# quarkquartet/nuSIprop

Measured on AMD Instinct MI355X. Metric: full propagations/sec at N_E=300, 1 & 8 GPU; achieved HBM GB/s on cascade kernel, higher is better.
Workload: dtype f64

## Files before the change

nusiprop_amd/csrc/nusi_kernels.hip:

```cpp
#include <hip/hip_runtime.h>

#include <algorithm>
#include <cstdlib>
#include <vector>

#include "nusi_internal.hpp"

namespace nusi {


__device__ __attribute__((noinline)) void warn_entry(int* warn, int* wmin, int T, int p, int w, int n, int m)
{
    atomicOr(&warn[p], w);
    if (wmin)
#pragma unroll
        for (int b = 0; b < 4; ++b)
            if ((w >> b) & 1) atomicMin(&wmin[((size_t)p * 4 + b) * T + n], m);
}

constexpr int kGaWaves = 4;
constexpr int kGaTerms = kAlphatSlots;
struct LdsSink {
    double* v;
    double* r;
// ... 152 lines not shown
    if (n >= T) return;
    const Point& P = pts[p];
    if (!P.non_resonant) return;
    double v[2];
    int f;
    const int nv = ga_pre_slot(P, k, g.lo[n], g.hi[n], slot, v, &f);
    double* o = pre + ((size_t)(p * 3 + k) * kGaPreFields + f) * T + n;
    o[0] = v[0];
    if (nv == 2) o[T] = v[1];
}

size_t gamma_alphat_pre_doubles(int T, int npts) { return (size_t)3 * kGaPreFields * T * npts; }

hipError_t launch_gamma_alphat(const GridDev& g, const Point* pts, int npts, const SplineSet* spl, TablesDev t,
                               int* warn, hipStream_t s, bool ref)
{
    dim3 grid((g.T + 62) / 63, npts, 2);
    if (ref && t.Gpre) {
        hipLaunchKernelGGL(k_ga_dilogs, dim3((g.T + 63) / 64, npts, 3 * kGaPreSlots), dim3(64), 0, s, g, pts, t.Gpre);
        hipLaunchKernelGGL((k_gamma_alphat<true, 2, true>), grid, dim3(384), 0, s, g, pts, spl, t.G, t.At, warn, t.Wmin,
                           t.Gpre);
        return hipGetLastError();
    }
    if (npts <= 16) {
        if (ref) hipLaunchKernelGGL((k_gamma_alphat<true, 2>), grid, dim3(384), 0, s, g, pts, spl, t.G, t.At, warn, t.Wmin);
        else hipLaunchKernelGGL((k_gamma_alphat<false, 2>), grid, dim3(384), 0, s, g, pts, spl, t.G, t.At, warn, t.Wmin);
    } else {
        if (ref) hipLaunchKernelGGL((k_gamma_alphat<true, 1>), grid, dim3(192), 0, s, g, pts, spl, t.G, t.At, warn, t.Wmin);
        else hipLaunchKernelGGL((k_gamma_alphat<false, 1>), grid, dim3(192), 0, s, g, pts, spl, t.G, t.At, warn, t.Wmin);
    }
    return hipGetLastError();
}


__host__ __device__ constexpr int alpha_tile_lds_doubles(int cs, int ct, int G)
{
    return alpha_tile_corner_block(cs, ct, G) + alpha_tile_edge_doubles(cs, ct, G) + (G > 1 ? G * kTileThreads : 0);
}

constexpr int kTileWaves = 3;
#define NUSI_TILE_ATTR __attribute__((amdgpu_waves_per_eu(kTileWaves, kTileWaves)))
template <int G, bool kRef>
__global__ __launch_bounds__(kTileThreads) NUSI_TILE_ATTR void k_alpha_tile(GridDev g, const Point* __restrict__ pts, const SplineSet* __restrict__ splp,
                                                           const int* __restrict__ tiles, int cs_max, int ct_max,
                                                           const int* __restrict__ batches,
                                                           double* __restrict__ A, int* __restrict__ warn,
                                                           int* __restrict__ wmin)
{
    extern __shared__ __attribute__((aligned(16))) double sm[];
    const SplineSet& spl = *splp;
    __shared__ double tE[2 * kAlphaTile], sE[2 * kAlphaTile];
    __shared__ int tl[kAlphaTile], th[kAlphaTile], sl[kAlphaTile], sh[kAlphaTile];
    __shared__ int cnt[2];
    __shared__ double elo[2][kAlphaTile], ehi[2][kAlphaTile];
    const int tid = threadIdx.x, T = g.T;
    const int bw = batches ? batches[blockIdx.y] : (int)blockIdx.y | (1 << 24);
    const int p0 = bw & 0xffffff, nb = (G == 1) ? 1 : bw >> 24;
    const AlphaTile tile = alpha_tile_decode(tiles + kTileWords * blockIdx.x);
    const int n0 = tile.n0, m0 = tile.m0;
    const int Tm = (m0 + tile.mcnt < T) ? m0 + tile.mcnt : T;
    const int Tn = (n0 + tile.ncnt < T) ? n0 + tile.ncnt : T;
    const Point& P = pts[p0];
    if (tid < 2 * kAlphaTile) {
        const int side = tid / kAlphaTile, j = tid - side * kAlphaTile, b = (side ? m0 : n0) + j;
        if (b < (side ? Tm : Tn)) { elo[side][j] = g.lo[b]; ehi[side][j] = g.hi[b]; }
    }
    __syncthreads();
    if (tid == 0) cnt[0] = alpha_edge_list(elo[0], ehi[0], 0, Tn - n0, tE, tl, th);
    if (tid == 64) cnt[1] = alpha_edge_list(elo[1], ehi[1], 0, Tm - m0, sE, sl, sh);
    __syncthreads();
    const int ct = cnt[0], cs = cnt[1], cc = cs * ct;
    const int ln = tid % kAlphaTile, lm = tid / kAlphaTile;
    const int n = n0 + ln, m = m0 + lm;
    const bool valid = alpha_tile_slot_valid(tile, T, tid);
    if (cs > cs_max || ct > ct_max || nb > G) {
        if (valid)
            for (int q = 0; q < nb; ++q) A[(size_t)(p0 + q) * g.PT + (size_t)m * (m - 1) / 2 + n] = __builtin_nan("");
        return;
    }
    const bool nonres = P.non_resonant, maj = P.majorana;
    const bool needed = valid && (nonres || m == n + 1);
    double* cor = sm;
    double* edg = sm + alpha_tile_corner_block(cs, ct, G);
    double* tsum = edg + alpha_tile_edge_doubles(cs, ct, G);
    double tot1 = 0.0;
    {
        const int per = ct + cs + kAlphaTile, w = tid >> 6, l = tid & 63;
        int job = -1;
        if (3 * ct <= 64 && 3 * cs <= 128) {
            if (w == 0) { if (l < 3 * ct) job = (l / ct) * per + l % ct; }
            else if (w <= 2) { const int q = tid - 64; if (q < 3 * cs) job = (q / cs) * per + ct + q % cs; }
            else if (l < 3 * kAlphaTile) job = (l / kAlphaTile) * per + ct + cs + l % kAlphaTile;
        } else if (tid < 3 * per) {
            job = tid;
        }
        if (job >= 0) {
            alpha_tile_edge_job(P, job, tE, ct, sE, cs, g.lo, g.hi, m0, Tm, edg);
#pragma unroll 1
            for (int q = 0; q < nb; ++q)
                alpha_tile_edge_member_job(pts[p0 + q], q, G, job, tE, ct, sE, cs, g.lo, g.hi, m0, Tm, edg);
        }
        if (G > 1)
            for (int q = 0; q < nb; ++q) tsum[q * kTileThreads + tid] = 0.0;
    }
    for (int k = 0; k < 3; ++k) {
        __syncthreads();
        if (nonres && maj) {
            const double* edgk = edg + k * alpha_tile_edge_stride(cs, ct);
            for (int j = tid; j < cc; j += kTileThreads) {
                alpha_tile_corner_job<kRef>(j, edgk, ct, cs, cor);
#pragma unroll 1
                for (int q = 0; q < nb; ++q) alpha_tile_corner_member_job<kRef>(pts[p0 + q], q, j, edgk, ct, cs, cor);
            }
            for (int j = tid; j < kAlphaTile * (cs + ct); j += kTileThreads)
                alpha_tile_mixed_job(j, edgk, ct, cs, G, tl, th, sl, sh, n0, m0, Tn, Tm, cor);
        }
        __syncthreads();
        if (needed) {
            AlphaPre pre;
            const bool share = G > 1 && nb > 1 && nonres && maj;
            if (share) {
                const TileLeaves lv0 = alpha_tile_leaves(cor, edg, k, 0, G, cs, ct, lm, sl, sh, tl, th, ln);
                alpha_k_pre(P, k, g.lo[n], g.hi[n], g.lo[m], g.hi[m], lv0, pre);
            }
#pragma unroll 1
            for (int q = 0; q < nb; ++q) {
                double tot = (G > 1) ? tsum[q * kTileThreads + tid] : tot1;
                int w = 0;
                const TileLeaves lv = alpha_tile_leaves(cor, edg, k, q, G, cs, ct, lm, sl, sh, tl, th, ln);
                alpha_k(pts[p0 + q], spl, k, g.lo[n], g.hi[n], g.lo[m], g.hi[m], lv, tot, w, share ? &pre : nullptr);
                if (G > 1) tsum[q * kTileThreads + tid] = tot;
                else tot1 = tot;
                if (w) warn_entry(warn, wmin, T, p0 + q, w, n, m);
            }
        }
    }
    if (valid)
        for (int q = 0; q < nb; ++q)
            A[(size_t)(p0 + q) * g.PT + (size_t)m * (m - 1) / 2 + n] =
                needed ? ((G > 1) ? tsum[q * kTileThreads + tid] : tot1) : 0.0;
}

constexpr int kBatchQC = 5;
__host__ __device__ inline int alpha_batch_lds_doubles()
{
    const int c1 = kAlphaTile + 1;
    return (3 + kXFields + 2) * c1 * c1 + alpha_tile_edge_stride(c1, c1) +
           kBatchQC * alpha_batch_memb_doubles(c1, c1);
}
static_assert(kXFields * (kAlphaTile + 1) * (kAlphaTile + 1) >= 4 * (kAlphaTile + 1) * (kAlphaTile + 1) + kAlphaTile * 2 * (kAlphaTile + 1),
              "the bracket phase's blocks fit X");
static_assert(kBatchQC * (2 * (kAlphaTile + 1) + kAlphaTile) <= kTileThreads, "one member-edge round per chunk");
static_assert(3 + kBatchQC <= kXFields, "(kRef) the chunk's A fields fit X beside Dcr, Dci");

constexpr int kBatchWaves = 4, kBatchWavesRefo = 3;
constexpr int batch_waves(bool pp, bool ref) { return ref && !pp ? kBatchWavesRefo : kBatchWaves; }
#define NUSI_BCOLD __device__ __attribute__((noinline))
template <bool kRef>
NUSI_BCOLD void b_corner(int j, const double* edgk, int ct, int cs, double* per, double* tmp)
{
    alpha_batch_corner_job<kRef>(j, edgk, ct, cs, per, tmp);
}
NUSI_BCOLD double b_marg(double S, double t, double gr) { return alpha_member_ref_arg(S, t, gr); }
NUSI_BCOLD void b_xshared(int j, const double* edgk, int ct, int cs, double* X) { alpha_batch_xshared_job(j, edgk, ct, cs, X); }
NUSI_FN SplitLeaves batch_bracket_leaves(const double* P3, const double* tmp, const double* mix, const double* edgk,
                                         int cs, int ct, int lm, int ln, int s0, int s1, int t0, int t1)
{
    const int cc = cs * ct;
    SplitLeaves lv;
    lv.cf[0] = P3; lv.cf[1] = tmp; lv.cf[2] = tmp + kCC; lv.cf[3] = tmp + 2 * kCC; lv.cf[4] = tmp + 3 * kCC;
    lv.cf[5] = P3 + kCC; lv.cf[6] = P3 + 2 * kCC;
    lv.corm = P3;
    lv.cc = cc; lv.ct = ct; lv.cs = cs; lv.mb = lm; lv.nb = ln;
    lv.sidx[0] = s0; lv.sidx[1] = s1; lv.tidx[0] = t0; lv.tidx[1] = t1;
    lv.ted = edgk; lv.sed = edgk + kTEdgeFields * ct; lv.mbv = lv.sed + kSEdgeFields * cs;
    lv.tedm = P3; lv.sedm = P3; lv.mbm = P3; lv.marg = P3;
    lv.xl = mix; lv.yl = mix + kAlphaTile * cs;
    return lv;
}
NUSI_BCOLD AlphaPre b_pre(const Point& P, int k, double Em, double Ep, double Emp, double Epp, const double* P3,
                          const double* tmp, const double* mix, const double* edgk, int cs, int ct, int lm, int ln,
                          int s0, int s1, int t0, int t1)
{
    const SplitLeaves lv = batch_bracket_leaves(P3, tmp, mix, edgk, cs, ct, lm, ln, s0, s1, t0, t1);
    AlphaPre pre;
    alpha_k_pre(P, k, Em, Ep, Emp, Epp, lv, pre);
    return pre;
}

__global__ __launch_bounds__(256) void k_alpha_medge(GridDev g, const Point* __restrict__ pts, double* __restrict__ med)
{
    const int j = blockIdx.x * 256 + threadIdx.x, p = blockIdx.y, k = blockIdx.z, T = g.T;
    if (j >= 5 * T) return;
    alpha_medge_job(pts[p], k, j, T, g.lo, g.hi, med + ((size_t)p * 3 + k) * kMedFields * T);
}

constexpr int kMcJobs = 1024;
__global__ __launch_bounds__(256) void k_alpha_mcorner(const Point* __restrict__ pts, const int* __restrict__ batches,
                                                       MCornerDev mc, int pc0, int jobs)
{
    __shared__ double v[2 * kMcJobs];
    __shared__ double cst[2][kMcJobs];
    const int bw = batches[blockIdx.y], k = blockIdx.z, tid = threadIdx.x;
    const int p0 = bw & 0xffffff, nb = (int)((unsigned)bw >> 24);
    const Point& P = pts[p0];
    if (!(P.non_resonant && P.majorana)) return;
    const int cb = jobs / nb;
    const long long c0 = (long long)blockIdx.x * cb;
    if (c0 >= mc.NC) return;
    const int nj = cb * nb;
    for (int cl = tid; cl < cb && c0 + cl < mc.NC; cl += 256) alpha_mcorner_st(P, k, c0 + cl, mc.ue, cst[0][cl], cst[1][cl]);
    __syncthreads();
    for (int j = tid; j < nj; j += 256) {
        const int cl = j / nb, q = j - cl * nb;
        if (c0 + cl >= mc.NC) break;
        const double S = cst[0][cl], t = cst[1][cl], gr = pts[p0 + q].a_gr;
        const cd Dc = alpha_member_ref_dc_inl(S, t, gr);
        v[2 * (q * cb + cl)] = Dc.r;
        v[2 * (q * cb + cl) + 1] = Dc.i;
    }
    __syncthreads();
    double* const o = mc.buf + (size_t)(p0 - pc0) * 6 * mc.NC + (size_t)k * 2 * nb * mc.NC;
    for (int e = tid; e < 2 * nj; e += 256) {
        const int q = e / (2 * cb), r = e - q * 2 * cb;
        if (c0 + r / 2 < mc.NC) o[((size_t)q * mc.NC + c0) * 2 + r] = v[e];
    }
}

void mcorner_edges(int T, const double* lo, const double* hi, std::vector<int>& eu, std::vector<double>& ue)
{
    eu.assign(2 * (size_t)T, 0);
    ue.clear();
    for (int b = 0; b < T; ++b) {
        if (b == 0 || !(lo[b] == hi[b - 1])) ue.push_back(lo[b]);
        eu[2 * b] = (int)ue.size() - 1;
        ue.push_back(hi[b]);
        eu[2 * b + 1] = (int)ue.size() - 1;
    }
}


#ifdef NUSI_BATCH_TRACE
constexpr int kBtWg = 16, kBtN = 512;
__device__ unsigned long long g_bt[kBtWg * 4 * kBtN];
#define NUSI_BT()                                                                                                   \
    do {                                                                                                            \
        if (kRef && !kPP && !kSplit && kPair == 1 && blockIdx.x < 4 && blockIdx.y < 4 && (threadIdx.x & 63) == 0 && bt_i < kBtN) \
            g_bt[((blockIdx.y * 4 + blockIdx.x) * 4 + (threadIdx.x >> 6)) * kBtN + bt_i] = __builtin_amdgcn_s_memtime(); \
        ++bt_i;                                                                                                     \
    } while (0)
#else
#define NUSI_BT() do { } while (0)
#endif
template <bool kPP, bool kRef, bool kSplit, int kPair>
__device__ __forceinline__ void alpha_batch_body(const GridDev& g, const Point* __restrict__ pts, const SplineSet* __restrict__ splp,
                                                 const int* __restrict__ tiles, const int* __restrict__ batches,
                                                 double* __restrict__ A, const double* __restrict__ med,
                                                 int* __restrict__ warn, int* __restrict__ wmin, const MCornerDev& mc,
                                                 int pc0, double* __restrict__ kt)
{
    static_assert(kPair == 1 || (kPair == 2 && kRef && !kPP && !kSplit), "paired points: the reference order without phi-phi");
    constexpr int kQC = kPair == 2 ? 4 : kBatchQC;
    extern __shared__ __attribute__((aligned(16))) double sm[];
    const SplineSet& spl = *splp;
    __shared__ double tE[2 * kAlphaTile], sE[2 * kAlphaTile];
    __shared__ int tl[kAlphaTile], th[kAlphaTile], sl[kAlphaTile], sh[kAlphaTile];
    __shared__ int cnt[2];
    __shared__ double elo[2][kAlphaTile], ehi[2][kAlphaTile];
    __shared__ unsigned char elist[kPair == 2 ? kPairEntries : 1];
    const int tid = threadIdx.x, T = g.T;
    const int bx = blockIdx.x, by = blockIdx.y;
    const int bw = batches[by];
    const int p0 = bw & 0xffffff, nb = (int)((unsigned)bw >> 24);
    const AlphaTile tile = alpha_tile_decode(tiles + kTileWords * bx);
    const int n0 = tile.n0, m0 = tile.m0;
    const int Tm = (m0 + tile.mcnt < T) ? m0 + tile.mcnt : T;
    const int Tn = (n0 + tile.ncnt < T) ? n0 + tile.ncnt : T;
    const Point& P = pts[p0];
    if (kPair == 2) {
        const int r = alpha_tile_entry_rank(tile, T, tid);
        if (r >= 0 && r < kPairEntries) elist[r] = (unsigned char)tid;
    }
    if (tid < 2 * kAlphaTile) {
        const int side = tid / kAlphaTile, j = tid - side * kAlphaTile, b = (side ? m0 : n0) + j;
        if (b < (side ? Tm : Tn)) { elo[side][j] = g.lo[b]; ehi[side][j] = g.hi[b]; }
    }
    __syncthreads();
    if (tid == 0) cnt[0] = alpha_edge_list(elo[0], ehi[0], 0, Tn - n0, tE, tl, th);
    if (tid == 64) cnt[1] = alpha_edge_list(elo[1], ehi[1], 0, Tm - m0, sE, sl, sh);
    __syncthreads();
    const int ct = cnt[0], cs = cnt[1], cc = cs * ct;
    __shared__ int tsrc[2 * kAlphaTile], ssrc[2 * kAlphaTile];
    if (tid < 2 * kAlphaTile) {
        const int side = tid / kAlphaTile, j = tid - side * kAlphaTile, b0 = side ? m0 : n0;
        const int* il = side ? sl : tl;
        const int* ih = side ? sh : th;
        int* src = side ? ssrc : tsrc;
        if (b0 + j < (side ? Tm : Tn)) {
            src[ih[j]] = 2 * (b0 + j) + 1;
            if (j == 0 || il[j] != ih[j - 1]) src[il[j]] = 2 * (b0 + j);
        }
    }
    const int hq = kPair == 2 ? __builtin_amdgcn_readfirstlane(tid / kPairEntries) : 0;
    const int nent = kPair == 2 ? alpha_tile_entries(tile, T) : 0;
    int slot = tid;
    if (kPair == 2) {
        const int e = tid % kPairEntries;
        slot = (e < nent && nent <= kPairEntries) ? elist[e] : kTileThreads - 1;
    }
    const int ln = slot % kAlphaTile, lm = slot / kAlphaTile;
    const int n = n0 + ln, m = m0 + lm;
    const bool valid = alpha_tile_slot_valid(tile, T, slot);
    const size_t eidx = (size_t)m * (m - 1) / 2 + n;
    if (cs > kAlphaTile + 1 || ct > kAlphaTile + 1 || (kPair == 2 && nent > kPairEntries)) {
        if (alpha_tile_slot_valid(tile, T, tid)) {
            const int md = m0 + tid / kAlphaTile;
            for (int q = 0; q < nb; ++q)
                A[(size_t)(p0 + q) * g.PT + (size_t)md * (md - 1) / 2 + n0 + tid % kAlphaTile] = __builtin_nan("");
        }
        return;
    }
    const bool nonres = P.non_resonant, maj = P.majorana, cornered = nonres && maj;
    const bool needed = valid && (nonres || m == n + 1);
    constexpr int ccmax = kCC;
    double* P3 = sm;
    double* X = P3 + 3 * ccmax;
    double* mem = X + kXFields * ccmax;
    double* edgk = mem + 2 * ccmax;
    double* membq = edgk + alpha_tile_edge_stride(kAlphaTile + 1, kAlphaTile + 1);
    const int mbd = alpha_batch_memb_doubles(cs, ct);
    double* tmp = X;
    double* mix = X + 4 * kCC;
    const int mjobs = ct + cs + kAlphaTile;
    int wsh = 0;
    const int kb = kSplit ? (int)blockIdx.z : 0, ke = kSplit ? kb + 1 : 3;
#ifdef NUSI_BATCH_TRACE
    int bt_i = 0;
#endif
#pragma unroll 1
    for (int k = kb; k < ke; ++k) {
        NUSI_BT();
        __syncthreads();
        if (tid < mjobs) alpha_tile_edge_job_k(P, k, tid, tE, ct, sE, cs, g.lo, g.hi, m0, Tm, edgk);
        __syncthreads();
        NUSI_BT();
        AlphaPre pre{};
        PPTerm ppt{0.0, 1.0, 1.0};
        if (cornered) {
            for (int j = tid; j < cc; j += kTileThreads) b_corner<kRef>(j, edgk, ct, cs, P3, tmp);
            for (int j = tid; j < kAlphaTile * (cs + ct); j += kTileThreads)
                alpha_batch_mixed_job(j, edgk, ct, cs, tl, th, sl, sh, n0, m0, Tn, Tm, mix, mix + kAlphaTile * cs);
            __syncthreads();
            NUSI_BT();
            if (needed) {
                pre = b_pre(P, k, g.lo[n], g.hi[n], g.lo[m], g.hi[m], P3, tmp, mix, edgk, cs, ct, lm, ln, sl[lm], sh[lm],
                            tl[ln], th[ln]);
                if (kPP) {
                    const SplitLeaves lv = batch_bracket_leaves(P3, tmp, mix, edgk, cs, ct, lm, ln, sl[lm], sh[lm],
                                                                tl[ln], th[ln]);
                    ppt = alpha_k_pp(P, spl, k, g.lo[n], g.hi[n], g.lo[m], g.hi[m], lv, wsh);
                }
            }
            __syncthreads();
            NUSI_BT();
            if (!kRef)
                for (int j = tid; j < cc; j += kTileThreads) b_xshared(j, edgk, ct, cs, X);
        }
        const bool reload = !kSplit && k > 0 && needed;
        double tnext = reload && hq < nb ? A[(size_t)(p0 + hq) * g.PT + eidx] : 0.0;
        const int mq = tid / mjobs, mjob = tid - mq * mjobs;
        const double2* const mcb =
            kRef ? reinterpret_cast<const double2*>(mc.buf + (size_t)(p0 - pc0) * 6 * mc.NC + (size_t)k * 2 * nb * mc.NC)
                 : nullptr;
        int moff = -1;
        double2 mcv = make_double2(0.0, 0.0), mcv2 = mcv;
        if (kRef && cornered && tid < cc) {
            const int si = tid / ct, ti = tid - si * ct;
            const int us = mc.eu[ssrc[si]], ut = mc.eu[tsrc[ti]];
            if (ut <= us) {
                moff = us * (us + 1) / 2 + ut;
                mcv = mcb[moff];
                if (kPair == 2 && nb > 1) mcv2 = mcb[mc.NC + moff];
            }
        }
#pragma unroll 1
        for (int q0 = 0; q0 < nb; q0 += kQC) {
            const int nq = (nb - q0 < kQC) ? nb - q0 : kQC;
            __syncthreads();
            NUSI_BT();
            if (mq < nq) {
                MedVals mv{};
                alpha_batch_medge_load(nonres, mjob, tsrc, ct, ssrc, cs, m0, Tm, T,
                                       med + ((size_t)(p0 + q0 + mq) * 3 + k) * kMedFields * T, mv);
                alpha_batch_medge_store(nonres, mjob, ct, cs, m0, Tm, mv, membq + mq * mbd);
            }
            if (kRef && moff >= 0) {
                const int si = tid / ct, ti = tid - si * ct;
                const double S = edgk[kTEdgeFields * ct + kSEdgeVal * cs + si], t = edgk[kTEdgeVal * ct + ti];
#pragma unroll 1
                for (int qq = 0; qq < nq; ++qq)
                    X[(3 + qq) * kCC + tid] =
                        kPP ? b_marg(S, t, pts[p0 + q0 + qq].a_gr) : alpha_member_ref_arg(S, t, pts[p0 + q0 + qq].a_gr);
            }
            NUSI_BT();
#pragma unroll 1
            for (int qq = 0; qq < nq; qq += kPair) {
                const int q = q0 + qq + hq;
                const bool act = kPair == 1 || q < nb;
                const Point& Q = pts[p0 + (act ? q : nb - 1)];
                const double* memb = membq + (qq + hq) * mbd;
                double tot = tnext;
                if (reload && q + kPair < nb) tnext = A[(size_t)(p0 + q + kPair) * g.PT + eidx];
                __syncthreads();
                NUSI_BT();
                if (cornered) {
                    if (kRef) {
                        if (moff >= 0) {
                            const size_t o = (size_t)(q0 + qq) * mc.NC + moff;
                            X[tid] = mcv.x; X[kCC + tid] = mcv.y;
                            if (kPair == 2) { mem[tid] = mcv2.x; mem[kCC + tid] = mcv2.y; }
                            if (q0 + qq + kPair < nb) mcv = mcb[o + kPair * mc.NC];
                            if (kPair == 2 && q0 + qq + 3 < nb) mcv2 = mcb[o + 3 * mc.NC];
                        }
                    }
                    else
                        for (int j = tid; j < cc; j += kTileThreads) alpha_batch_mcorner_job(Q, j, edgk, ct, cs, X, memb, mem);
                }
                __syncthreads();
                NUSI_BT();
                int w = 0;
                TermRec rec;
                if (needed && act) {
                    SplitLeavesT<kRef> lv;
                    lv.cf[0] = P3; lv.cf[1] = P3; lv.cf[2] = P3; lv.cf[3] = P3; lv.cf[4] = P3;
                    lv.cf[5] = P3 + kCC; lv.cf[6] = P3 + 2 * kCC;
                    lv.corm = kRef && hq == 0 ? X : mem;
                    lv.cc = cc; lv.ct = ct; lv.cs = cs; lv.mb = lm; lv.nb = ln;
                    lv.sidx[0] = sl[lm]; lv.sidx[1] = sh[lm]; lv.tidx[0] = tl[ln]; lv.tidx[1] = th[ln];
                    lv.ted = edgk; lv.sed = edgk + kTEdgeFields * ct; lv.mbv = lv.sed + kSEdgeFields * cs;
                    lv.tedm = memb; lv.sedm = memb + ct; lv.mbm = memb + ct + 2 * cs;
                    lv.marg = kRef ? X + (3 + qq + hq) * kCC : memb + ct + 2 * cs + kAlphaTile + 2 * ct;
                    lv.xl = mix; lv.yl = mix;
                    if (kSplit)
                        alpha_k<SplitLeavesT<kRef>, kPP>(Q, spl, k, g.lo[n], g.hi[n], g.lo[m], g.hi[m], lv, rec, w,
                                                         cornered ? &pre : nullptr, kPP && cornered ? &ppt : nullptr);
                    else
                        alpha_k<SplitLeavesT<kRef>, kPP>(Q, spl, k, g.lo[n], g.hi[n], g.lo[m], g.hi[m], lv, tot, w,
                                                         cornered ? &pre : nullptr, kPP && cornered ? &ppt : nullptr);
                }
                if (kSplit) {
                    if (valid) {
                        double* o = kt + ((((size_t)(p0 + q) * 3 + k) * g.PT + eidx) << 3);
#pragma unroll
                        for (int j = 0; j < 7; ++j) o[j] = rec.v[j];
                        o[7] = needed ? (double)rec.n : -1.0;
                    }
                } else if (valid && act) A[(size_t)(p0 + q) * g.PT + eidx] = needed ? tot : 0.0;
                if (w) warn_entry(warn, wmin, T, p0 + q, w, n, m);
                NUSI_BT();
            }
        }
    }
    if (wsh)
        for (int q = 0; q < nb; ++q) warn_entry(warn, wmin, T, p0 + q, wsh, n, m);
}
template <bool kPP, bool kRef, bool kSplit = false>
__global__ __launch_bounds__(kTileThreads) __attribute__((amdgpu_waves_per_eu(batch_waves(kPP, kRef), batch_waves(kPP, kRef))))
void k_alpha_batch(GridDev g, const Point* __restrict__ pts, const SplineSet* __restrict__ splp, const int* __restrict__ tiles,
                   const int* __restrict__ batches, double* __restrict__ A, const double* __restrict__ med,
                   int* __restrict__ warn, int* __restrict__ wmin, MCornerDev mc, int pc0, double* __restrict__ kt)
{
    if (!kPP && kRef && !kSplit && alpha_tile_decode(tiles + kTileWords * blockIdx.x).pair) {
        alpha_batch_body<false, true, false, 2>(g, pts, splp, tiles, batches, A, med, warn, wmin, mc, pc0, nullptr);
        return;
    }
    alpha_batch_body<kPP, kRef, kSplit, 1>(g, pts, splp, tiles, batches, A, med, warn, wmin, mc, pc0, kt);
}

__global__ __launch_bounds__(kTileThreads) void k_alpha_ksum(GridDev g, const int* __restrict__ tiles,
                                                             const int* __restrict__ batches, const double* __restrict__ kt,
                                                             double* __restrict__ A)
{
    const int tid = threadIdx.x, T = g.T;
    const int bw = batches[blockIdx.y];
    const int p0 = bw & 0xffffff, nb = (int)((unsigned)bw >> 24);
    const AlphaTile tile = alpha_tile_decode(tiles + kTileWords * blockIdx.x);
    const int n = tile.n0 + tid % kAlphaTile, m = tile.m0 + tid / kAlphaTile;
    if (!alpha_tile_slot_valid(tile, T, tid)) return;
    const size_t eidx = (size_t)m * (m - 1) / 2 + n;
    for (int q = 0; q < nb; ++q) {
        double tot = 0.0;
        bool skip = false;
        for (int k = 0; k < 3; ++k) {
            const double* o = kt + ((((size_t)(p0 + q) * 3 + k) * g.PT + eidx) << 3);
            const int cnt = (int)o[7];
            if (cnt < 0) skip = true;
            for (int j = 0; j < cnt; ++j) tot += o[j];
        }
        A[(size_t)(p0 + q) * g.PT + eidx] = skip ? 0.0 : tot;
    }
}

__global__ __launch_bounds__(256) void k_table_shift(int T, long long PT, int Tb, long long PTb, const int2* __restrict__ map,
                                                     int s0, TablesDev tb, TablesDev t, int* __restrict__ warn)
{
    const int q = blockIdx.y, s = s0 + q;
    const int bi = map[q].x, o = map[q].y;
    const long long e = (long long)blockIdx.x * 256 + threadIdx.x;
    if (e < T) {
        t.G[(size_t)s * T + e] = tb.G[(size_t)bi * Tb + e + o];
        t.At[(size_t)s * T + e] = tb.At[(size_t)bi * Tb + e + o];
        int bits = 0;
#pragma unroll
        for (int b = 0; b < 4; ++b)
            if (tb.Wmin[((size_t)bi * 4 + b) * Tb + e + o] <= T - 1 + o) bits |= 1 << b;
        if (bits) atomicOr(&warn[s], bits);
    }
    if (e >= PT) return;
    int m = (int)((1.0 + sqrt(1.0 + 8.0 * (double)e)) * 0.5);
    while ((long long)m * (m - 1) / 2 > e) --m;
    while ((long long)(m + 1) * m / 2 <= e) ++m;
    const long long n = e - (long long)m * (m - 1) / 2, mb = m + o;
    t.A[(size_t)s * PT + e] = tb.A[(size_t)bi * PTb + mb * (mb - 1) / 2 + n + o];
}

hipError_t launch_table_shift(const GridDev& g, const GridDev& gb, const int2* map, int s0, int nshift, TablesDev tb,
                              TablesDev t, int* warn, hipStream_t s)
{
    if (nshift <= 0) return hipSuccess;
    if (!tb.Wmin) return hipErrorInvalidValue;
    const long long ne = std::max<long long>(g.PT, g.T);
    hipLaunchKernelGGL(k_table_shift, dim3((unsigned)((ne + 255) / 256), nshift), dim3(256), 0, s, g.T, g.PT, gb.T, gb.PT,
                       map, s0, tb, t, warn);
    return hipGetLastError();
}

hipError_t alpha_tiles_create(int T, const unsigned char* shared, AlphaTilesDev* out)
{
    const AlphaTileList tl = alpha_tiles_build(T, shared);
    const int cap_core = kAlphaTile + 1, cap_ext = 2 * kAlphaTile;
    const int csm[3] = {cap_core, cap_ext, cap_ext}, ctm[3] = {cap_core, cap_core, cap_ext};
    std::vector<int> all;
    for (int c = 0; c < 3; ++c) {
        out->ncls[c] = tl.count(c);
        out->cs_max[c] = csm[c];
        out->ct_max[c] = ctm[c];
        all.insert(all.end(), tl.cls[c].begin(), tl.cls[c].end());
    }
    hipError_t e = hipMalloc(&out->tiles, sizeof(int) * std::max<size_t>(1, all.size()));
    if (e != hipSuccess) return e;
    return hipMemcpy(out->tiles, all.data(), sizeof(int) * all.size(), hipMemcpyHostToDevice);
}

void alpha_tiles_destroy(AlphaTilesDev* t)
{
    if (t->tiles) (void)hipFree(t->tiles);
    t->tiles = nullptr;
}

static thread_local const char* t_alpha_kernel = "";
const char* last_alpha_kernel() { return t_alpha_kernel; }

template <bool kRef>
static hipError_t launch_alpha_t(const GridDev& g, const Point* pts, int npts, const SplineSet* spl,
                                 const AlphaTilesDev& at, TablesDev t, int* warn, hipStream_t s, const int* batches,
                                 int nbatches, int gmax, int kernel, int nb_plain, const int* h_batches,
                                 const MCornerDev* mc)
{
    t_alpha_kernel = kRef ? "k_alpha_tile[refo]" : "k_alpha_tile";
    if (kernel == 0 && batches) {
        t_alpha_kernel = kRef ? "k_alpha_mcorner + k_alpha_batch[refo]" : "k_alpha_batch";
        int off = 0;
        for (int c = 0; c < 3; ++c) {
            if (at.ncls[c] == 0) continue;
            const int cs = at.cs_max[c], ct = at.ct_max[c];
            if (c == 0) {
                const size_t lds = sizeof(double) * (size_t)alpha_batch_lds_doubles();
                if (cs > kAlphaTile + 1 || ct > kAlphaTile + 1) return hipErrorInvalidValue;
                {
                    if (!t.Med) return hipErrorInvalidValue;
                    hipLaunchKernelGGL(k_alpha_medge, dim3((unsigned)((5 * g.T + 255) / 256), npts, 3), dim3(256), 0, s,
                                       g, pts, t.Med);
                }
                const bool split = t.Kt && nb_plain == nbatches;
                if (!kRef) {
                    if (split) {
                        hipLaunchKernelGGL((k_alpha_batch<false, false, true>), dim3(at.ncls[0], nbatches, 3),
                                           dim3(kTileThreads), lds, s, g, pts, spl, at.tiles, batches, t.A, t.Med, warn,
                                           t.Wmin, MCornerDev{}, 0, t.Kt);
                        hipLaunchKernelGGL(k_alpha_ksum, dim3(at.ncls[0], nbatches), dim3(kTileThreads), 0, s, g, at.tiles,
                                           batches, t.Kt, t.A);
                    } else if (nb_plain > 0)
                        hipLaunchKernelGGL((k_alpha_batch<false, false>), dim3(at.ncls[0], nb_plain), dim3(kTileThreads),
                                           lds, s, g, pts, spl, at.tiles, batches, t.A, t.Med, warn, t.Wmin, MCornerDev{}, 0, nullptr);
                    if (nbatches > nb_plain)
                        hipLaunchKernelGGL((k_alpha_batch<true, false>), dim3(at.ncls[0], nbatches - nb_plain),
                                           dim3(kTileThreads), lds, s, g, pts, spl, at.tiles, batches + nb_plain, t.A,
                                           t.Med, warn, t.Wmin, MCornerDev{}, 0, nullptr);
                } else {
                    if (!mc || !mc->buf || !h_batches) return hipErrorInvalidValue;
                    for (int b = 0; b < nbatches;) {
                        const int lim = b < nb_plain ? nb_plain : nbatches, pc0 = h_batches[b] & 0xffffff;
                        int e = b, ntb = 0, nbmax = 0;
                        while (e < lim) {
                            const int nbe = (int)((unsigned)h_batches[e] >> 24);
                            if (e > b && ntb + nbe > mc->cap_tables) break;
                            ntb += nbe;
                            nbmax = std::max(nbmax, nbe);
                            ++e;
                        }
                        if (ntb > mc->cap_tables) return hipErrorInvalidValue;
// ... 85 lines not shown
```

nusiprop_amd/csrc/nusi_physics.hpp:

```cpp
#pragma once

#include "nusi_math.hpp"
#include "nusi_spline.hpp"
#include "nusi_alpha_tiles.hpp"

#define NUSI_MASS_LOOP _Pragma("unroll 1")

namespace nusi {

struct Point {
    double mphi, g, mntot, si, norm;
    double norm_total;
    double Ga;
    double mn[3];
    double u[3];
    double U2[9];
    int majorana, non_resonant, phiphi, source;
    int tslot;
    double a_wgt[3];
    double a_s;
    double a_st;
    double a_nrm;
    double a_gr;
};
// ... 1182 lines not shown
         + SSP * (l2m * (lSp + Lmq) - l2p * (lSm + Lpq) + Lmp * (mc.lr - Lmq + Lpq))
         + SSP * ((lSp + Lmm) * (fSm.lS2 + Lmt - lam) + (lSm + Lpm) * (l2p - Lmt + lam))
         + SS * (mc.lr2 + Lmq - Lpq) * (2 * tm + Pq * lap)
         + SSP * (cmm.G - cpm.G - cmq.G + cpq.G)
         + SSP * (Fp + Fm));
}
template <class Lv>
NUSI_FN void alpha_k_pre(const Point& P, int k, double Em, double Ep, double Emp, double Epp, const Lv& lv, AlphaPre& pre)
{
    const double mphi = P.mphi, m2 = mphi * mphi, m4 = (mphi * mphi) * (mphi * mphi), mk = P.mn[k];
    const double tp = lv.tval(1, mk, Ep, m2), tm = lv.tval(0, mk, Em, m2);
    const double Sp = lv.Sval(1, mk, Epp, m2), Sm = lv.Sval(0, mk, Emp, m2);
    alpha_bracket_t(lv, Sm, Sp, tm, tp, m4, pre.Dt, pre.Bt);
    alpha_bracket_tu(lv, Sm, Sp, tm, tp, m4, pre.Dtu, pre.Btu);
}
template <class Lv>
NUSI_FN PPTerm alpha_k_pp(const Point& P, const SplineSet& spl, int k, double Em, double Ep, double Emp, double Epp,
                          const Lv& lv, int& warn)
{
    const double mphi = P.mphi, m2 = mphi * mphi, mk = P.mn[k];
    const double tp = lv.tval(1, mk, Ep, m2), tm = lv.tval(0, mk, Em, m2);
    const double Sp = lv.Sval(1, mk, Epp, m2), Sm = lv.Sval(0, mk, Emp, m2);
    if (!(Sm > 4 && P.phiphi)) return PPTerm{0.0, 1.0, 1.0};
    const AlphaSEdge eSm = lv.sedge(0, Sm), eSp = lv.sedge(1, Sp);
    const PPTerm X = alpha_phiphi_core(spl, Sm, Sp, tm, tp, eSm.lS, eSp.lS);
    warn |= X.oob;
    return X;
}

struct TermRec {
    double v[7];
    int n = 0;
    NUSI_FN TermRec& operator+=(double x)
    {
        v[n++] = x;
        return *this;
    }
};
template <class Lv, bool kPhiPhi = true, class Acc = double>
NUSI_FN void alpha_k(const Point& P, const SplineSet& spl, int k, double Em, double Ep, double Emp, double Epp,
                     const Lv& lv, Acc& tot, int& warn, const AlphaPre* pre = nullptr, const PPTerm* ppt = nullptr)
{
    const double g = P.g, mphi = P.mphi;
    const double g4 = (g * g) * (g * g), m2 = mphi * mphi, m4 = (mphi * mphi) * (mphi * mphi);
    const double gr = P.a_gr, gr2 = gr * gr;
    const bool maj = P.majorana;
    const double mk = P.mn[k], uk = P.u[k];
    const double tp = lv.tval(1, mk, Ep, m2), tm = lv.tval(0, mk, Em, m2);
    const double Sp = lv.Sval(1, mk, Epp, m2), Sm = lv.Sval(0, mk, Emp, m2);
    const double wgt = P.a_wgt[k];
    const AlphaMBin mb = lv.mbin(Sm, Sp);

    double as;
    if (Sp < 1e-5)
        as = P.a_s * (tm - tp) *
             ((gr * (1 + gr2 + 2 * Sm)) / ((1 + gr2) * (1 + gr2)) * (Sp - Sm) + gr / ((1 + gr2) * (1 + gr2)) * ((Sp - Sm) * (Sp - Sm)));
    else
        as = P.a_s * (tm - tp) * mb.atd;
    as *= uk;
    if (!maj) as /= 2.;
    tot += wgt * as;
    if (!P.non_resonant) return;

    const AlphaTEdge eTm = lv.tedge(0, tm), eTp = lv.tedge(1, tp);
    const AlphaSEdge eSm = lv.sedge(0, Sm), eSp = lv.sedge(1, Sp);
    const double Lmt = eTm.Lm1, Lmp = eTp.Lm1;
    const double lSm = eSm.lS, lSp = eSp.lS;
    double at, au, atu = 0., ast;
    if (maj) {
        {
            double D, B;
            if (pre) { D = pre->Dt; B = pre->Bt; }
            else alpha_bracket_t(lv, Sm, Sp, tm, tp, m4, D, B);
            at = g4 / D * B;
            if (at < 0) at = gl33_rect(0, tp, tm, Sm, Sp) * (g4 / (16 * kPi * m4));
            at *= uk;
            tot += wgt * at;
            au = at;
            tot += wgt * au;
        }
        NUSI_PHASE();
        {
            double D, B;
            if (pre) { D = pre->Dtu; B = pre->Btu; }
            else alpha_bracket_tu(lv, Sm, Sp, tm, tp, m4, D, B);
            atu = g4 / D * B;
            atu *= uk;
            tot += wgt * atu;
        }
        NUSI_PHASE();
        {
            const AlphaCorner cmm = lv.corner(0, 0, Sm, tm), cpm = lv.corner(1, 0, Sp, tm);
            const AlphaCorner cmq = lv.corner(0, 1, Sm, tp), cpq = lv.corner(1, 1, Sp, tp);
            const AlphaSEdge fSm = lv.sedge(0, Sm), fSp = lv.sedge(1, Sp);
            const AlphaTEdge fTm = lv.tedge(0, tm), fTp = lv.tedge(1, tp);
            const double Lmm = cmm.L, Lpm = cpm.L, Lmq = cmq.L, Lpq = cpq.L;
            const double lSm = fSm.lS, lSp = fSp.lS, Lmt = fTm.Lm1, Lmp = fTp.Lm1;
            const double Lsm = fSm.Ls, Lsp = fSp.Ls;
            const double cm = fTm.cm, cp = fTp.cm;
            const double L2m = fTm.L2, L2p = fTp.L2;
            const double am = fTm.am, ap = fTp.am;
            ast = P.a_st *
                  (2 * gr * (cmm.Dri - cmm.Dci - cpm.Dri + cpm.Dci - cmq.Dri + cmq.Dci + cpq.Dri - cpq.Dci)
                   - 2 * (cmm.Drr - cmm.Dcr - cpm.Drr + cpm.Dcr - cmq.Drr + cmq.Dcr + cpq.Drr - cpq.Dcr)
                   + 2 * gr * (cm - cmm.A) * Lmm
                   - 2 * gr * (cm - cpm.A) * Lpm
                   + 2 * gr * (cp - cpq.A) * Lpq
                   - 2 * gr * (cp - cmq.A) * Lmq
                   + 2 * (gr * fSm.cS - gr * fSp.cS + Lsp / 2. - Lsm / 2. + lSm - lSp) * (2 * (tm - tp) + (Lmt - Lmp))
                   + Lmm * (Lsm - L2m - 2 * (lSm - am)) - Lpm * (Lsp - L2m - 2 * (lSp - am))
                   - Lmq * (Lsm - L2p - 2 * (lSm - ap)) + Lpq * (Lsp - L2p - 2 * (lSp - ap)));
        }
        NUSI_PHASE();
    } else {
        const double brk = -((tm - tp) * (2 + tm * (-1 + tp) - tp)) - 2 * (-1 + tm) * (-1 + tp) * (Lmt - Lmp);
        at = 3. / 2. * g4 / (32 * kPi * m4 * Sm * Sp * (-1 + tm) * (-1 + tp)) * (Sm - Sp) * brk;
        if (at < 0) at = gl33_rect(1, tp, tm, Sm, Sp) * (3. / 2. * g4 / (32 * kPi * m4));
        at *= uk;
        tot += wgt * at;
        au = 1. / 2. * g4 / (32 * kPi * m4 * Sm * Sp * (-1 + tm) * (-1 + tp)) * (Sm - Sp) * brk;
        if (au < 0) au = gl33_rect(1, tp, tm, Sm, Sp) * (1. / 2. * g4 / (32 * kPi * m4));
        au *= uk;
        tot += wgt * au;
        tot += wgt * atu;
        const double Lsm = eSm.Ls, Lsp = eSp.Ls;
        ast = P.a_st *
              ((2 * gr * eSm.cS - 2 * gr * eSp.cS + 2 * lSm - 2 * lSp + Lsp - Lsm) * (tm - tp + Lmt - Lmp));
    }
    ast *= uk;
    tot += wgt * ast;
    const double asu = maj ? ast : 0.;
    tot += wgt * asu;

    double app = 0.0;
    if (kPhiPhi && Sm > 4 && P.phiphi)
    {
        PPTerm X;
        if (ppt) X = *ppt;
        else {
            X = alpha_phiphi_core(spl, Sm, Sp, tm, tp, lSm, lSp);
            warn |= X.oob;
        }
        app = alpha_phiphi_scale(P, uk, X);
    }
    tot += wgt * app;

    const double nrm = P.a_nrm;
    const double sst = ast + as + at;
    if (as < 0 || ((at < 0 || au < 0 || atu < 0 || sst < 0) &&
                   (at / nrm < -1e-11 || au / nrm < -1e-11 || atu / nrm < -1e-11 || sst / nrm < -1e-11)))
        warn |= kWarnAlpha;
}

template <bool kRef = false>
NUSI_FN double alpha_entry(const Point& P, const SplineSet& spl, double Em, double Ep, double Emp, double Epp, int& warn)
{
    const DirectLeavesT<kRef> lv{P.Ga / P.mphi, (P.Ga / P.mphi) * (P.Ga / P.mphi), P.mphi, P.Ga};
    double tot = 0;
    NUSI_MASS_LOOP
    for (int k = 0; k < 3; ++k) alpha_k(P, spl, k, Em, Ep, Emp, Epp, lv, tot, warn);
    return tot;
}

}
```

Before: 63460.

## Stage chunk corner values in LDS and evaluate two points per pass

On the reference, non-phi-phi path, each chunk's corner Dcr/Dci values and member arguments are now staged into LDS for every point up front. This removes the two block barriers that previously ran per point. When possible, two consecutive points are evaluated together by a new fused alpha_k_two routine that shares the bracket computation and interleaves both points' term phases. This is meant to cut synchronisation overhead and raise instruction-level parallelism. The costs are a smaller chunk size, more LDS use per chunk, and a specialised code path that must stay consistent with alpha_k (it assumes u-term equals t-term and no phi-phi term).

```diff
diff --git a/nusiprop_amd/csrc/nusi_kernels.hip b/nusiprop_amd/csrc/nusi_kernels.hip
--- a/nusiprop_amd/csrc/nusi_kernels.hip
+++ b/nusiprop_amd/csrc/nusi_kernels.hip
@@ -328,6 +328,9 @@
               "the bracket phase's blocks fit X");
 static_assert(kBatchQC * (2 * (kAlphaTile + 1) + kAlphaTile) <= kTileThreads, "one member-edge round per chunk");
 static_assert(3 + kBatchQC <= kXFields, "(kRef) the chunk's A fields fit X beside Dcr, Dci");
+constexpr int kStageQC = 4;
+static_assert(3 * kStageQC <= kXFields + 2, "(staged chunks) the chunk's Dcr, Dci, A fields fit X and the mem block after it");
+static_assert(kStageQC <= kBatchQC && kStageQC % 2 == 0, "the staged chunk fits memb, and a pair never straddles two");
 
 constexpr int kBatchWaves = 4, kBatchWavesRefo = 3;
 constexpr int batch_waves(bool pp, bool ref) { return ref && !pp ? kBatchWavesRefo : kBatchWaves; }
@@ -435,8 +438,9 @@
                                                  int* __restrict__ warn, int* __restrict__ wmin, const MCornerDev& mc,
                                                  int pc0, double* __restrict__ kt)
 {
-    static_assert(kPair == 1 || (kPair == 2 && kRef && !kPP && !kSplit), "paired points: the reference order without phi-phi");
-    constexpr int kQC = kPair == 2 ? 4 : kBatchQC;
+    constexpr bool kStage = kRef && !kPP && !kSplit;
+    static_assert(kPair == 1 || (kPair == 2 && kStage), "paired points: the reference order without phi-phi");
+    constexpr int kQC = kStage ? kStageQC : kBatchQC;
     extern __shared__ __attribute__((aligned(16))) double sm[];
     const SplineSet& spl = *splp;
     __shared__ double tE[2 * kAlphaTile], sE[2 * kAlphaTile];
@@ -549,14 +553,13 @@
             kRef ? reinterpret_cast<const double2*>(mc.buf + (size_t)(p0 - pc0) * 6 * mc.NC + (size_t)k * 2 * nb * mc.NC)
                  : nullptr;
         int moff = -1;
-        double2 mcv = make_double2(0.0, 0.0), mcv2 = mcv;
+        double2 mcv = make_double2(0.0, 0.0);
         if (kRef && cornered && tid < cc) {
             const int si = tid / ct, ti = tid - si * ct;
             const int us = mc.eu[ssrc[si]], ut = mc.eu[tsrc[ti]];
             if (ut <= us) {
                 moff = us * (us + 1) / 2 + ut;
-                mcv = mcb[moff];
-                if (kPair == 2 && nb > 1) mcv2 = mcb[mc.NC + moff];
+                if (!kStage) mcv = mcb[moff];
             }
         }
 #pragma unroll 1
@@ -574,50 +577,68 @@
                 const int si = tid / ct, ti = tid - si * ct;
                 const double S = edgk[kTEdgeFields * ct + kSEdgeVal * cs + si], t = edgk[kTEdgeVal * ct + ti];
 #pragma unroll 1
-                for (int qq = 0; qq < nq; ++qq)
-                    X[(3 + qq) * kCC + tid] =
-                        kPP ? b_marg(S, t, pts[p0 + q0 + qq].a_gr) : alpha_member_ref_arg(S, t, pts[p0 + q0 + qq].a_gr);
+                for (int qq = 0; qq < nq; ++qq) {
+                    if (kStage) {
+                        const double2 v = mcb[(size_t)(q0 + qq) * mc.NC + moff];
+                        const double a = alpha_member_ref_arg(S, t, pts[p0 + q0 + qq].a_gr);
+                        double* const f = X + 3 * qq * kCC + tid;
+                        f[0] = v.x; f[kCC] = v.y; f[2 * kCC] = a;
+                    } else
+                        X[(3 + qq) * kCC + tid] =
+                            kPP ? b_marg(S, t, pts[p0 + q0 + qq].a_gr) : alpha_member_ref_arg(S, t, pts[p0 + q0 + qq].a_gr);
+                }
             }
             NUSI_BT();
+            if (kStage) __syncthreads();
 #pragma unroll 1
-            for (int qq = 0; qq < nq; qq += kPair) {
+            for (int qq = 0, step = kPair; qq < nq; qq += step) {
                 const int q = q0 + qq + hq;
                 const bool act = kPair == 1 || q < nb;
                 const Point& Q = pts[p0 + (act ? q : nb - 1)];
                 const double* memb = membq + (qq + hq) * mbd;
+                const bool two = kStage && kPair == 1 && cornered && qq + hq + kPair < nq;
+                step = two ? 2 * kPair : kPair;
                 double tot = tnext;
-                if (reload && q + kPair < nb) tnext = A[(size_t)(p0 + q + kPair) * g.PT + eidx];
-                __syncthreads();
-                NUSI_BT();
-                if (cornered) {
-                    if (kRef) {
-                        if (moff >= 0) {
-                            const size_t o = (size_t)(q0 + qq) * mc.NC + moff;
-                            X[tid] = mcv.x; X[kCC + tid] = mcv.y;
-                            if (kPair == 2) { mem[tid] = mcv2.x; mem[kCC + tid] = mcv2.y; }
-                            if (q0 + qq + kPair < nb) mcv = mcb[o + kPair * mc.NC];
-                            if (kPair == 2 && q0 + qq + 3 < nb) mcv2 = mcb[o + 3 * mc.NC];
+                double tot2 = two && reload ? A[(size_t)(p0 + q + kPair) * g.PT + eidx] : 0.0;
+                if (reload && q + step < nb) tnext = A[(size_t)(p0 + q + step) * g.PT + eidx];
+                if (!kStage) {
+                    __syncthreads();
+                    NUSI_BT();
+                    if (cornered) {
+                        if (kRef) {
+                            if (moff >= 0) {
+                                const size_t o = (size_t)(q0 + qq) * mc.NC + moff;
+                                X[tid] = mcv.x; X[kCC + tid] = mcv.y;
+                                if (q0 + qq + 1 < nb) mcv = mcb[o + mc.NC];
+                            }
                         }
+                        else
+                            for (int j = tid; j < cc; j += kTileThreads) alpha_batch_mcorner_job(Q, j, edgk, ct, cs, X, memb, mem);
                     }
-                    else
-                        for (int j = tid; j < cc; j += kTileThreads) alpha_batch_mcorner_job(Q, j, edgk, ct, cs, X, memb, mem);
+                    __syncthreads();
+                    NUSI_BT();
                 }
-                __syncthreads();
-                NUSI_BT();
-                int w = 0;
+                int w = 0, w2 = 0;
                 TermRec rec;
                 if (needed && act) {
                     SplitLeavesT<kRef> lv;
                     lv.cf[0] = P3; lv.cf[1] = P3; lv.cf[2] = P3; lv.cf[3] = P3; lv.cf[4] = P3;
                     lv.cf[5] = P3 + kCC; lv.cf[6] = P3 + 2 * kCC;
-                    lv.corm = kRef && hq == 0 ? X : mem;
+                    lv.corm = kStage ? X + 3 * (qq + hq) * kCC : kRef ? X : mem;
                     lv.cc = cc; lv.ct = ct; lv.cs = cs; lv.mb = lm; lv.nb = ln;
                     lv.sidx[0] = sl[lm]; lv.sidx[1] = sh[lm]; lv.tidx[0] = tl[ln]; lv.tidx[1] = th[ln];
                     lv.ted = edgk; lv.sed = edgk + kTEdgeFields * ct; lv.mbv = lv.sed + kSEdgeFields * cs;
                     lv.tedm = memb; lv.sedm = memb + ct; lv.mbm = memb + ct + 2 * cs;
-                    lv.marg = kRef ? X + (3 + qq + hq) * kCC : memb + ct + 2 * cs + kAlphaTile + 2 * ct;
+                    lv.marg = kStage ? X + (3 * (qq + hq) + 2) * kCC
+                              : kRef ? X + (3 + qq) * kCC : memb + ct + 2 * cs + kAlphaTile + 2 * ct;
                     lv.xl = mix; lv.yl = mix;
-                    if (kSplit)
+                    if (kStage && two) {
+                        SplitLeavesT<kRef> lv2 = lv;
+                        lv2.corm = lv.corm + 3 * kPair * kCC; lv2.marg = lv.marg + 3 * kPair * kCC;
+                        lv2.tedm = lv.tedm + kPair * mbd; lv2.sedm = lv.sedm + kPair * mbd; lv2.mbm = lv.mbm + kPair * mbd;
+                        alpha_k_two(Q, pts[p0 + q + kPair], k, g.lo[n], g.hi[n], g.lo[m], g.hi[m], lv, lv2, tot, tot2, w, w2, pre);
+                    }
+                    else if (kSplit)
                         alpha_k<SplitLeavesT<kRef>, kPP>(Q, spl, k, g.lo[n], g.hi[n], g.lo[m], g.hi[m], lv, rec, w,
                                                          cornered ? &pre : nullptr, kPP && cornered ? &ppt : nullptr);
                     else
@@ -631,8 +652,12 @@
                         for (int j = 0; j < 7; ++j) o[j] = rec.v[j];
                         o[7] = needed ? (double)rec.n : -1.0;
                     }
-                } else if (valid && act) A[(size_t)(p0 + q) * g.PT + eidx] = needed ? tot : 0.0;
+                } else if (valid && act) {
+                    A[(size_t)(p0 + q) * g.PT + eidx] = needed ? tot : 0.0;
+                    if (kStage && two) A[(size_t)(p0 + q + kPair) * g.PT + eidx] = needed ? tot2 : 0.0;
+                }
                 if (w) warn_entry(warn, wmin, T, p0 + q, w, n, m);
+                if (kStage && w2) warn_entry(warn, wmin, T, p0 + q + kPair, w2, n, m);
                 NUSI_BT();
             }
         }
diff --git a/nusiprop_amd/csrc/nusi_physics.hpp b/nusiprop_amd/csrc/nusi_physics.hpp
--- a/nusiprop_amd/csrc/nusi_physics.hpp
+++ b/nusiprop_amd/csrc/nusi_physics.hpp
@@ -1358,6 +1358,100 @@
         warn |= kWarnAlpha;
 }
 
+template <class Lv>
+NUSI_FN void alpha_k_two(const Point& Pa, const Point& Pb, int k, double Em, double Ep, double Emp, double Epp,
+                         const Lv& la, const Lv& lb, double& tota, double& totb, int& warna, int& warnb,
+                         const AlphaPre& pre)
+{
+    struct Pt { double g4, m4, gr, uk, wgt, as, at, atu, ast; };
+    const double m2a = Pa.mphi * Pa.mphi, mka = Pa.mn[k];
+    const double tp = la.tval(1, mka, Ep, m2a), tm = la.tval(0, mka, Em, m2a);
+    const double Sp = la.Sval(1, mka, Epp, m2a), Sm = la.Sval(0, mka, Emp, m2a);
+    auto head = [&](const Point& P, const Lv& lv, Pt& s, double& tot) {
+        const double g = P.g, mphi = P.mphi;
+        s.g4 = (g * g) * (g * g);
+        s.m4 = (mphi * mphi) * (mphi * mphi);
+        s.gr = P.a_gr;
+        const double gr = s.gr, gr2 = gr * gr;
+        s.uk = P.u[k];
+        s.wgt = P.a_wgt[k];
+        const AlphaMBin mb = lv.mbin(Sm, Sp);
+        double as;
+        if (Sp < 1e-5)
+            as = P.a_s * (tm - tp) *
+                 ((gr * (1 + gr2 + 2 * Sm)) / ((1 + gr2) * (1 + gr2)) * (Sp - Sm) + gr / ((1 + gr2) * (1 + gr2)) * ((Sp - Sm) * (Sp - Sm)));
+        else
+            as = P.a_s * (tm - tp) * mb.atd;
+        as *= s.uk;
+        s.as = as;
+        tot += s.wgt * as;
+    };
+    auto tu = [&](Pt& s, double& tot) {
+        double at = s.at;
+        at *= s.uk;
+        s.at = at;
+        tot += s.wgt * at;
+        tot += s.wgt * at;
+    };
+    auto tuu = [&](Pt& s, double& tot) {
+        double atu = s.g4 / pre.Dtu * pre.Btu;
+        atu *= s.uk;
+        s.atu = atu;
+        tot += s.wgt * atu;
+    };
+    auto st = [&](const Point& P, const Lv& lv, Pt& s) {
+        const double gr = s.gr;
+        const AlphaCorner cmm = lv.corner(0, 0, Sm, tm), cpm = lv.corner(1, 0, Sp, tm);
+        const AlphaCorner cmq = lv.corner(0, 1, Sm, tp), cpq = lv.corner(1, 1, Sp, tp);
+        const AlphaSEdge fSm = lv.sedge(0, Sm), fSp = lv.sedge(1, Sp);
+        const AlphaTEdge fTm = lv.tedge(0, tm), fTp = lv.tedge(1, tp);
+        const double Lmm = cmm.L, Lpm = cpm.L, Lmq = cmq.L, Lpq = cpq.L;
+        const double lSm = fSm.lS, lSp = fSp.lS, Lmt = fTm.Lm1, Lmp = fTp.Lm1;
+        const double Lsm = fSm.Ls, Lsp = fSp.Ls;
+        const double cm = fTm.cm, cp = fTp.cm;
+        const double L2m = fTm.L2, L2p = fTp.L2;
+        const double am = fTm.am, ap = fTp.am;
+        s.ast = P.a_st *
+                (2 * gr * (cmm.Dri - cmm.Dci - cpm.Dri + cpm.Dci - cmq.Dri + cmq.Dci + cpq.Dri - cpq.Dci)
+                 - 2 * (cmm.Drr - cmm.Dcr - cpm.Drr + cpm.Dcr - cmq.Drr + cmq.Dcr + cpq.Drr - cpq.Dcr)
+                 + 2 * gr * (cm - cmm.A) * Lmm
+                 - 2 * gr * (cm - cpm.A) * Lpm
+                 + 2 * gr * (cp - cpq.A) * Lpq
+                 - 2 * gr * (cp - cmq.A) * Lmq
+                 + 2 * (gr * fSm.cS - gr * fSp.cS + Lsp / 2. - Lsm / 2. + lSm - lSp) * (2 * (tm - tp) + (Lmt - Lmp))
+                 + Lmm * (Lsm - L2m - 2 * (lSm - am)) - Lpm * (Lsp - L2m - 2 * (lSp - am))
+                 - Lmq * (Lsm - L2p - 2 * (lSm - ap)) + Lpq * (Lsp - L2p - 2 * (lSp - ap)));
+    };
+    auto tail = [&](const Point& P, Pt& s, double& tot, int& warn) {
+        double ast = s.ast;
+        ast *= s.uk;
+        tot += s.wgt * ast;
+        tot += s.wgt * ast;
+        const double app = 0.0;
+        tot += s.wgt * app;
+        const double nrm = P.a_nrm, as = s.as, at = s.at, au = s.at, atu = s.atu;
+        const double sst = ast + as + at;
+        if (as < 0 || ((at < 0 || au < 0 || atu < 0 || sst < 0) &&
+                       (at / nrm < -1e-11 || au / nrm < -1e-11 || atu / nrm < -1e-11 || sst / nrm < -1e-11)))
+            warn |= kWarnAlpha;
+    };
+    Pt a, b;
+    head(Pa, la, a, tota); head(Pb, lb, b, totb);
+    a.at = a.g4 / pre.Dt * pre.Bt; b.at = b.g4 / pre.Dt * pre.Bt;
+    if (a.at < 0 || b.at < 0) {
+        const double r = gl33_rect(0, tp, tm, Sm, Sp);
+        if (a.at < 0) a.at = r * (a.g4 / (16 * kPi * a.m4));
+        if (b.at < 0) b.at = r * (b.g4 / (16 * kPi * b.m4));
+    }
+    tu(a, tota); tu(b, totb);
+    NUSI_PHASE();
+    tuu(a, tota); tuu(b, totb);
+    NUSI_PHASE();
+    st(Pa, la, a); st(Pb, lb, b);
+    NUSI_PHASE();
+    tail(Pa, a, tota, warna); tail(Pb, b, totb, warnb);
+}
+
 template <bool kRef = false>
 NUSI_FN double alpha_entry(const Point& P, const SplineSet& spl, double Em, double Ep, double Emp, double Epp, int& warn)
 {
```

After: 68220, median of 6. 1.08x the previous value.
